# als244/ResNet

Hardware: AMD Instinct MI355X
Metric: images/sec ResNet-50 fp32 224x224 batch256 (higher is better)
Workload: dtype f32

## Files before the change

### include/resnet_mi.h

```cpp
#ifndef RESNET_MI_H
#define RESNET_MI_H
#include <stddef.h>
#include <stdint.h>

#ifdef __cplusplus
extern "C" {
#endif

typedef struct {
    char **labels;
    char **synsets;
    int *counts;
    int n_classes;
} Class_Metadata;

typedef struct {
    int input;
    int init_kernel_dim;
    int init_conv_filters;
    int init_conv_stride;
    int init_maxpool_dim;
    int init_maxpool_stride;
    int n_conv_blocks;
    int *is_block_spatial_reduction;
// ... 218 lines not shown
int mi_op_avgpool_fwd(const float *x, float *y, int N, int C, int H);
int mi_op_avgpool_bwd(const float *dy, float *dx, int N, int C, int H);
int mi_op_relu_deriv(const float *x, const float *up, float *out, size_t n);
int mi_op_matmul(const float *A, const float *B, float *out, int m, int k, int n);
int mi_op_matmul_lt(const float *A_kxm, const float *B, float *out, int m, int k, int n);
int mi_op_matmul_rt(const float *A, const float *B_nxk, float *out, int m, int k, int n);
int mi_op_softmax(const float *x, float *out, int N, int L);
int mi_op_ce_deriv(const float *pred, const int *labels, float *d, int N, int L);
int mi_op_adam(float *p, const float *g, float *m, float *v, size_t n, float lr, float wd, float b1, float b2,
               float cur_b1, float cur_b2, float eps, int *nan_flag_dev);
int mi_op_nhwc_to_nchw(const float *in, float *out, int N, int H, int W, int C);
int mi_debug_lds_fill(uint32_t word);
int mi_debug_poison_lds(void);
int mi_debug_lds_probe(uint32_t word, size_t out[4]);
int mi_debug_lds_geometry(size_t out[3]);
int mi_debug_lds_fill_mode(int on, uint32_t word);
size_t mi_debug_lds_fills(void);
int mi_debug_redzone(size_t zone_bytes, int fill_byte);
int mi_debug_redzone_check(void);
void mi_debug_redzone_stats(size_t *allocs_checked, size_t *zone_bytes_checked, size_t *live);
int mi_debug_trace_names(char *buf, size_t cap);
void mi_debug_trace_clear(void);
int mi_debug_conv_plan(int op, int N, int C, int H, int K, int k, int stride, int out[9]);
int mi_op_fill_uniform(float *out, size_t n, uint64_t seed, float lo, float hi);
enum { MI_ROUTE_DEFAULT = 0, MI_ROUTE_CL = 1, MI_ROUTE_CL2 = 2, MI_ROUTE_PW = 3 };
int mi_conv_plan(int dtype, int route, int op, int N, int C, int H, int K, int k, int stride, int out[7]);
enum { MI_FWD_F32, MI_FWD_BF16, MI_FWD_CL, MI_FWD_STEM_F32, MI_FWD_STEM_BF16, MI_FWD_PW  };
enum { MI_DG_F32, MI_DG_BF16, MI_DG_CL, MI_DG_CL2 };
enum { MI_WG_F32, MI_WG_BF16, MI_WG_CL, MI_WG_CL2, MI_WG_STEM_F32, MI_WG_STEM_BF16 };
int mi_layer_routes(int dtype, int policy, int N, int C, int H, int K, int k, int stride, int site, int out[4]);
enum {
    MI_K_NONE,
    MI_K_IGEMM,
    MI_K_GEMM1X1,
    MI_K_DCONV,
    MI_K_WGRADC,
    MI_K_WGRAD,
    MI_K_BGEMM,
    MI_K_PW_WGRAD,
    MI_K_CL_CONV,
    MI_K_CL_DGRAD2,
    MI_K_CL_WGRAD,
    MI_K_CL_WGRAD2,
    MI_K_ST32_FWD,
    MI_K_ST32_WGRAD,
    MI_K_ST_FWD,
// ... 183 lines not shown
```

### resnet_amd/binding.py

```python
import ctypes as C
import os

_HERE = os.path.dirname(os.path.abspath(__file__))
LIB_PATH = os.environ.get("RESNET_MI_LIB") or os.path.join(_HERE, "libresnet_mi.so")

_fp = C.POINTER(C.c_float)
_ip = C.POINTER(C.c_int)


class Dims(C.Structure):
    _fields_ = [("input", C.c_int), ("init_kernel_dim", C.c_int), ("init_conv_filters", C.c_int),
                ("init_conv_stride", C.c_int), ("init_maxpool_dim", C.c_int), ("init_maxpool_stride", C.c_int),
                ("n_conv_blocks", C.c_int), ("is_block_spatial_reduction", _ip), ("final_depth", C.c_int),
                ("output", C.c_int)]


class BatchNorm(C.Structure):
    _fields_ = [("spatial_dim", C.c_int), ("depth", C.c_int), ("gamma", _fp), ("beta", _fp)]


class ConvBlock(C.Structure):
    _fields_ = [("incoming_filters", C.c_int), ("incoming_spatial_dim", C.c_int), ("reduced_depth", C.c_int),
                ("expanded_depth", C.c_int), ("stride", C.c_int), ("depth_reduction", _fp),
                ("norm_depth_reduction", C.POINTER(BatchNorm)), ("spatial", _fp), ("norm_spatial", C.POINTER(BatchNorm)),
# ... 202 lines not shown
    "mi_op_avgpool_bwd": (_i, [_vp, _vp, _i, _i, _i]),
    "mi_op_relu_deriv": (_i, [_vp, _vp, _vp, _sz]),
    "mi_op_matmul": (_i, [_vp, _vp, _vp, _i, _i, _i]),
    "mi_op_matmul_lt": (_i, [_vp, _vp, _vp, _i, _i, _i]),
    "mi_op_matmul_rt": (_i, [_vp, _vp, _vp, _i, _i, _i]),
    "mi_op_softmax": (_i, [_vp, _vp, _i, _i]),
    "mi_op_ce_deriv": (_i, [_vp, _vp, _vp, _i, _i]),
    "mi_op_adam": (_i, [_vp, _vp, _vp, _vp, _sz, _f, _f, _f, _f, _f, _f, _f, _vp]),
    "mi_op_nhwc_to_nchw": (_i, [_vp, _vp, _i, _i, _i, _i]),
    "mi_op_fill_uniform": (_i, [_vp, _sz, _u64, _f, _f]),
    "mi_debug_poison_lds": (_i, []),
    "mi_debug_lds_fill": (_i, [C.c_uint32]),
    "mi_debug_lds_probe": (_i, [C.c_uint32, C.POINTER(_sz)]),
    "mi_debug_lds_geometry": (_i, [C.POINTER(_sz)]),
    "mi_debug_lds_fill_mode": (_i, [_i, C.c_uint32]),
    "mi_debug_lds_fills": (_sz, []),
    "mi_debug_redzone": (_i, [_sz, _i]),
    "mi_debug_redzone_check": (_i, []),
    "mi_debug_redzone_stats": (None, [C.POINTER(_sz)] * 3),
    "mi_debug_trace_names": (_i, [C.c_char_p, _sz]),
    "mi_debug_trace_clear": (None, []),
    "mi_debug_conv_plan": (_i, [_i] * 7 + [_vp]),
    "mi_conv_plan": (_i, [_i] * 9 + [_vp]),
    "mi_layer_routes": (_i, [_i] * 9 + [_vp]),
    "mi_layer_kernels": (_i, [_i] * 9 + [_vp]),
    "mi_debug_trainer_routes": (_i, [_T, _vp, _i]),
    "mi_trainer_set_dtype": (_i, [_T, _i]),
    "mi_trainer_get_dtype": (_i, [_T]),
    "mi_trainer_set_store_policy": (_i, [_T, _i]),
    "mi_trainer_activation_bytes": (_sz, [_T]),
    "mi_trainer_device_bytes": (_sz, [_T]),
    "mi_clear_error": (None, []),
    "mi_trainer_check_errors": (_i, [_T]),
    "mi_trainer_end_epoch": (None, [_T, _f, _f, _f]),
    "mi_trainer_set_optimizer": (_i, [_T, _i, _f, _f]),
    "mi_trainer_get_optimizer": (_i, [_T]),
    "mi_op_loss_head": (_i, [_vp, _vp, _vp, _vp, _vp, _vp, _i, _i, _f, _i, _vp, _vp]),
    "mi_trainer_set_loss": (_i, [_T, _f, _i, _i]),
    "mi_trainer_metrics": (_i, [_T, C.POINTER(MiLossMetrics), C.POINTER(MiLossMetrics), _i]),
    "mi_trainer_track_running_stats": (_i, [_T, _i, _f]),
    "mi_bn_unbias": (_f, [C.c_int64]),
    "mi_op_bn_running_update": (_i, [_vp, _vp, _vp, _vp, _i, _vp, _i, _f]),
    "mi_trainer_running_stats_channels": (_i, [_T]),
    "mi_trainer_get_running_stats": (_i, [_T, _vp, _vp]),
    "mi_trainer_set_running_stats": (_i, [_T, _vp, _vp]),
    "mi_trainer_running_updates": (C.c_int64, [_T]),
# ... 117 lines not shown
```

### resnet_amd/csrc/kernels_igemm.hip

```cpp
#include "mi_common.hpp"
#include <type_traits>
#include "mi_device.h"

typedef float f32x16 __attribute__((ext_vector_type(16)));
typedef float pf4 __attribute__((ext_vector_type(4)));

enum { IG_FWD = 0, IG_DGRAD = 1, IG_WGRAD = 2 };

struct IgArgs {
    int N, C, K, H, W, Ho, Wo;
    int HW, P;
    int ncols;
    int mtiles;
    int tiles;
    int ctiles;
    int klen;
    FastDiv fdP, fdWo, fdM;
    int full, tsplit, tklen, cpt;
    FastDiv fdTs, fdCpt;
    float *tailbuf;
    float *bn_part;
    int bn_np;
    const float *bnb_x, *bnb_mask, *bnb_mean;
    float *bnb_part;
// ... 21 lines not shown
    if (nv <= 0) { mean = 0.f; m2 = 0.f; }
}
__device__ __forceinline__ void ig_merge(float &na, float &ma, float &qa, float nb, float mb, float qb) {
    const float n = na + nb;
    if (n > 0.f) {
        const float dlt = mb - ma, f = nb / n;
        ma = ma + dlt * f;
        qa = qa + qb + dlt * dlt * na * f;
    }
    na = n;
}

#define IG_BK 32
#ifdef IG_STAMP
__device__ unsigned long long ig_stamps[8 * 16384];
#define IG_T(slot) do { if (threadIdx.x == 0 && blockIdx.x < 16384 && blockIdx.y == 0) ig_stamps[blockIdx.x * 8 + (slot)] = __builtin_amdgcn_s_memtime(); } while (0)
#else
#define IG_T(slot) do { } while (0)
#endif
#ifndef IG_ABLATE
#define IG_ABLATE 0
#endif

template <int MODE, int KS, int S, int WMW, bool VBP = false>
__global__ void __launch_bounds__(256)
igemm_kernel(const float *__restrict__ Aop, const float *__restrict__ Bop, float *__restrict__ Out,
             const float *__restrict__ addend, const IgArgs g) {
    constexpr int BM = 64 * WMW;
    constexpr int TN = WMW == 2 ? 2 : 1;
    constexpr int WNC = 32 * TN;
    constexpr int T = KS * KS, PAD = KS / 2;
    constexpr int LDA = (MODE == IG_WGRAD) ? BM + 1 : BM + 4;
    constexpr int LDB = (MODE == IG_WGRAD) ? 129 : 132;
    constexpr int NA4 = BM / 32;
    constexpr int NAS = BM / 8;
    constexpr bool VB = VBP && KS == 1 && MODE != IG_WGRAD;
    constexpr bool CT64 = VBP && MODE == IG_WGRAD;
    extern __shared__ __attribute__((aligned(16))) float ig_smem[];
    float *As = ig_smem;
    float *Bs = ig_smem + 2 * IG_BK * LDA;
    const int tid = threadIdx.x, lane = tid & 63;
    const int wave = __builtin_amdgcn_readfirstlane(tid >> 6);
    const int wm = WMW == 2 ? wave >> 1 : 0, wn = WMW == 2 ? wave & 1 : wave;

    IG_T(0);
    uint32_t L = blockIdx.x;
    int tail_id = -1, it0 = 0, nt_slice = 0;
    uint32_t wg_split = blockIdx.y;
    if (MODE != IG_WGRAD && g.tsplit > 1 && L >= (uint32_t)g.full) {
        tail_id = (int)(L - (uint32_t)g.full);
        const uint32_t tl = fd_div((uint32_t)tail_id, g.fdTs);
        const int z = tail_id - (int)tl * g.tsplit;
        L = (uint32_t)g.full + tl;
        it0 = z * g.tklen;
        nt_slice = g.tklen;
    } else if (MODE == IG_WGRAD && gridDim.y >= 8) {
        const uint32_t T_ = gridDim.x, tot = T_ * gridDim.y, per = tot >> 3;
        uint32_t V = blockIdx.y * T_ + blockIdx.x;
        if (V < per * 8) V = (V & 7) * per + (V >> 3);
        wg_split = V / T_;
        L = V - wg_split * T_;
    } else {
        const uint32_t lim = MODE != IG_WGRAD && g.tsplit > 1 ? (uint32_t)g.full : (uint32_t)g.tiles;
// ... 7 lines not shown
    f32x16 acc[2][TN];
#pragma unroll
    for (int i = 0; i < 2; i++)
#pragma unroll
        for (int j = 0; j < TN; j++)
#pragma unroll
            for (int r = 0; r < 16; r++) acc[i][j][r] = 0.f;

    uint32_t a_lane = 0, b_lane = 0;
    uint32_t mask = 0;
    int ph = 0, pw = 0, ntaps = 1;
    int wg_t = 0, wg_r = 0, wg_s = 0, cblk = 0, kend = 0;
    int ntiles = 0;
    if (MODE == IG_FWD || MODE == IG_DGRAD) {
        const int Mdim = MODE == IG_FWD ? g.K : g.C;
        const int a_i = (tid & (BM / 4 - 1)) * 4, a_k = tid / (BM / 4);
        a_lane = (uint32_t)(a_k * Mdim + a_i) * 4u;
        const int j = VB ? n0 + (tid & 31) * 4 : n0 + (tid & 127);
        const bool jin = j < g.ncols;
        const uint32_t jc = jin ? (uint32_t)j : (uint32_t)g.ncols - (VB ? 4u : 1u);
        const uint32_t n = fd_div(jc, g.fdP);
        const uint32_t p = jc - n * g.P;
        const uint32_t ho = fd_div(p, g.fdWo), wo = p - ho * g.Wo;
        const int b_k = VB ? (tid >> 5) : 16 * (tid >> 7);
        if (MODE == IG_FWD) {
            b_lane = (uint32_t)(n * g.C * g.HW + (S * ho) * g.W + S * wo + b_k * g.HW) * 4u;
#pragma unroll
            for (int t = 0; t < T; t++) {
                const int hi = S * (int)ho - PAD + t / KS, wi = S * (int)wo - PAD + t % KS;
                if (jin && hi >= 0 && hi < g.H && wi >= 0 && wi < g.W) mask |= 1u << t;
            }
            ntaps = T;
            ntiles = T * (g.C / IG_BK);
        } else if (S == 1) {
            b_lane = (uint32_t)(n * g.K * g.P + p + b_k * g.P) * 4u;
#pragma unroll
            for (int t = 0; t < T; t++) {
                const int hs = (int)ho + PAD - t / KS, ws = (int)wo + PAD - t % KS;
                if (jin && hs >= 0 && hs < g.Ho && ws >= 0 && ws < g.Wo) mask |= 1u << t;
            }
            ntaps = T;
            ntiles = T * (g.K / IG_BK);
        } else {
            const int cls = 3 - (int)blockIdx.y;
            ph = cls >> 1; pw = cls & 1;
            const int ntw = pw ? 2 : 1;
            ntaps = (ph ? 2 : 1) * ntw;
            b_lane = (uint32_t)(n * g.K * g.P + p + b_k * g.P) * 4u;
            for (int tt = 0; tt < ntaps; tt++) {
                const int th = tt / ntw, tw = tt - th * ntw;
                const int dh = (ph && th == 0) ? 1 : 0, dw = (pw && tw == 0) ? 1 : 0;
                if (jin && (int)ho + dh < g.Ho && (int)wo + dw < g.Wo) mask |= 1u << tt;
            }
            ntiles = ntaps * (g.K / IG_BK);
        }
    } else {
        if (CT64) { wg_t = 2 * (int)ct; cblk = 0; }
        else {
            wg_t = (int)(ct / (uint32_t)g.ctiles);
            cblk = (int)(ct - (uint32_t)wg_t * g.ctiles) * 128;
        }
        wg_r = wg_t / KS; wg_s = wg_t - KS * wg_r;
        const int kbeg = (int)wg_split * g.klen;
        kend = min(g.N * g.P, kbeg + g.klen);
        ntiles = (kend - kbeg + IG_BK - 1) / IG_BK;
    }

    pf4 ra4[NA4];
    float ra[NAS], rb[16];
    pf4 rb4[4];
    int sel_a = 1, sel_b = 1;
    int ld_t = 0, ld_c0 = 0;
    if (MODE != IG_WGRAD && tail_id >= 0) {
        ld_t = (int)fd_div((uint32_t)it0, g.fdCpt);
        ld_c0 = (it0 - ld_t * g.cpt) * IG_BK;
        ntiles = min(nt_slice, ntiles - it0);
    }
    int ld_k0 = (MODE == IG_WGRAD) ? (int)wg_split * g.klen : 0;
    const char *fa = nullptr, *fb = nullptr;
    uint32_t fa_lane = 0, fb_lane = 0;
    uint32_t fb_lane2 = 0;
    auto ldg = [](const char *ubase, uint32_t lane_off) -> float { return *(const float *)(ubase + lane_off); };
    auto ldg4 = [](const char *ubase, uint32_t lane_off) -> pf4 { return *(const pf4 *)(ubase + lane_off); };

    auto fetch_into = [&](const int p, pf4 *ra4, float *ra, float *rb, pf4 *rb4, int &sel_a, int &sel_b) {
        if (MODE == IG_FWD || MODE == IG_DGRAD) {
            if (p == 0) {
                const int t = min(ld_t, ntaps - 1);
                sel_b = (mask >> t) & 1;
                if (MODE == IG_FWD) {
                    const int r = KS == 3 ? (t * 11) >> 5 : 0, s = t - KS * r;
                    fa = (const char *)(Aop + (size_t)(t * g.C + ld_c0) * g.K + m0);
                    fb = (const char *)(Bop + (size_t)ld_c0 * g.HW);
                    fb_lane = b_lane + (uint32_t)(sel_b * ((r - PAD) * g.W + (s - PAD)) * 4);
                    ld_c0 += IG_BK;
                    if (ld_c0 == g.C) { ld_c0 = 0; ld_t++; }
                } else {
                    int wt, doff;
                    if (S == 1) {
                        const int r = KS == 3 ? (t * 11) >> 5 : 0, s = t - KS * r;
                        wt = t;
                        doff = (PAD - r) * g.Wo + (PAD - s);
                    } else {
                        const int th = pw ? t >> 1 : t, tw = pw ? t & 1 : 0;
                        const int r = ph ? 2 * th : 1, s = pw ? 2 * tw : 1;
                        wt = 3 * r + s;
                        doff = (ph & (th ^ 1)) * g.Wo + (pw & (tw ^ 1));
                    }
                    fa = (const char *)(Aop + (size_t)(wt * g.K + ld_c0) * g.C + m0);
                    fb = (const char *)(Bop + (size_t)ld_c0 * g.P);
                    fb_lane = b_lane + (uint32_t)(sel_b * doff * 4);
                    ld_c0 += IG_BK;
                    if (ld_c0 == g.K) { ld_c0 = 0; ld_t++; }
                }
            }
            const size_t bstride = (MODE == IG_FWD ? (size_t)g.HW : (size_t)g.P) * 4;
            const size_t astride = (MODE == IG_FWD ? (size_t)g.K : (size_t)g.C) * 4;
            if (VB) { if ((p & 1) == 0) rb4[p >> 1] = ldg4(fb + (size_t)(4 * p) * bstride, fb_lane); }
            else {
                rb[2 * p] = ldg(fb + (size_t)(2 * p) * bstride, fb_lane);
                rb[2 * p + 1] = ldg(fb + (size_t)(2 * p + 1) * bstride, fb_lane);
            }
            if (p % (8 / NA4) == 0) ra4[p / (8 / NA4)] = ldg4(fa + (size_t)(4 * p) * astride, a_lane);
        } else {
            if (p == 0) {
                const int kk = ld_k0 + (tid & 31);
                sel_a = kk < kend;
                const uint32_t kc = sel_a ? (uint32_t)kk : (uint32_t)kend - 1;
                const uint32_t n = fd_div_ge2(kc, g.fdP);
                const uint32_t pp = kc - n * g.P;
                const uint32_t ho = fd_div_ge2(pp, g.fdWo), wo = pp - ho * g.Wo;
                const int hi = S * (int)ho - PAD + wg_r, wi = S * (int)wo - PAD + wg_s;
                const int inb = (int)((uint32_t)hi < (uint32_t)g.H) & (int)((uint32_t)wi < (uint32_t)g.W);
                sel_b = sel_a & inb;
                const uint32_t row = (uint32_t)tid >> 5;
                fa = (const char *)(Aop + (size_t)m0 * g.P);
                fb = (const char *)(Bop + (size_t)cblk * g.HW);
                fa_lane = (n * (uint32_t)(g.K * g.P) + pp + row * g.P) * 4u;
                const uint32_t pix = inb ? (uint32_t)(hi * g.W + wi) : (S * ho) * g.W + S * wo;
                fb_lane = (n * (uint32_t)(g.C * g.HW) + pix + row * g.HW) * 4u;
                if (CT64) {
                    const int t1 = wg_t + 1, r1 = t1 / KS, s1 = t1 - KS * r1;
                    const int hj = S * (int)ho - PAD + r1, wj = S * (int)wo - PAD + s1;
                    const int inb1 = (int)((uint32_t)hj < (uint32_t)g.H) & (int)((uint32_t)wj < (uint32_t)g.W) & (int)(t1 < T);
                    const uint32_t pix1 = inb1 ? (uint32_t)(hj * g.W + wj) : (S * ho) * g.W + S * wo;
                    fb_lane2 = (n * (uint32_t)(g.C * g.HW) + pix1 + row * g.HW) * 4u;
                    sel_b |= (sel_a & inb1) << 1;
                }
                ld_k0 += IG_BK;
            }
            if (NAS == 16) {
                ra[2 * p] = ldg(fa + (size_t)(16 * p) * g.P * 4, fa_lane);
                ra[2 * p + 1] = ldg(fa + (size_t)(16 * p + 8) * g.P * 4, fa_lane);
            } else ra[p] = ldg(fa + (size_t)(8 * p) * g.P * 4, fa_lane);
            if (CT64) {
                rb[2 * p] = ldg(fb + (size_t)(16 * (p & 3)) * g.HW * 4, p < 4 ? fb_lane : fb_lane2);
                rb[2 * p + 1] = ldg(fb + (size_t)(16 * (p & 3) + 8) * g.HW * 4, p < 4 ? fb_lane : fb_lane2);
            } else {
                rb[2 * p] = ldg(fb + (size_t)(16 * p) * g.HW * 4, fb_lane);
                rb[2 * p + 1] = ldg(fb + (size_t)(16 * p + 8) * g.HW * 4, fb_lane);
            }
        }
    };
    auto fetch_part = [&](const int p) { fetch_into(p, ra4, ra, rb, rb4, sel_a, sel_b); };
    auto stash_from = [&](const int buf, const int p, const pf4 *ra4, const float *ra, const float *rb, const pf4 *rb4, const int sel_a, const int sel_b) {
        float *as = As + buf * IG_BK * LDA, *bs = Bs + buf * IG_BK * LDB;
        if (MODE == IG_WGRAD) {
            const int kx = tid & 31, row = tid >> 5;
            if (NAS == 16) {
                as[kx * LDA + row + 16 * p] = sel_a ? ra[2 * p] : 0.f;
                as[kx * LDA + row + 16 * p + 8] = sel_a ? ra[2 * p + 1] : 0.f;
            } else as[kx * LDA + row + 8 * p] = sel_a ? ra[p] : 0.f;
            const int sb = CT64 ? (sel_b >> (p >> 2)) & 1 : sel_b;
            bs[kx * LDB + row + 16 * p] = sb ? rb[2 * p] : 0.f;
            bs[kx * LDB + row + 16 * p + 8] = sb ? rb[2 * p + 1] : 0.f;
        } else {
            if (VB) {
                if ((p & 1) == 0) {
                    const pf4 z = {0.f, 0.f, 0.f, 0.f};
                    *(pf4 *)(bs + ((tid >> 5) + 4 * p) * LDB + (tid & 31) * 4) = sel_b ? rb4[p >> 1] : z;
                }
            } else {
                const int bj = tid & 127, b_k = 16 * (tid >> 7);
                bs[(b_k + 2 * p) * LDB + bj] = sel_b ? rb[2 * p] : 0.f;
                bs[(b_k + 2 * p + 1) * LDB + bj] = sel_b ? rb[2 * p + 1] : 0.f;
            }
            if (p % (8 / NA4) == 0) {
                const int a_i = (tid & (BM / 4 - 1)) * 4, a_k = tid / (BM / 4);
                *(pf4 *)(as + (a_k + 4 * p) * LDA + a_i) = ra4[p / (8 / NA4)];
            }
        }
    };
    auto stash_part = [&](const int buf, const int p) { stash_from(buf, p, ra4, ra, rb, rb4, sel_a, sel_b); };

    const int fr = lane & 31, fk = lane >> 5;
    {
        pf4 pa4[NA4], pb4[4];
        float pa[NAS], pb[16];
        int psel_a = 1, psel_b = 1;
#pragma unroll
        for (int p = 0; p < 8; p++) fetch_into(p, pa4, pa, pb, pb4, psel_a, psel_b);
#pragma unroll
        for (int p = 0; p < 8; p++) fetch_part(p);
#pragma unroll
        for (int p = 0; p < 8; p++) stash_from(0, p, pa4, pa, pb, pb4, psel_a, psel_b);
    }
    if (MODE == IG_WGRAD) {
#pragma unroll
        for (int q = 0; q < NAS; q++) asm volatile("" : "+v"(ra[q]));
    } else {
#pragma unroll
        for (int q = 0; q < NA4; q++) asm volatile("" : "+v"(ra4[q]));
    }
#pragma unroll
    for (int q = 0; q < 16; q++) { if (!VB) asm volatile("" : "+v"(rb[q])); }
#pragma unroll
    for (int q = 0; q < 4; q++) { if (VB) asm volatile("" : "+v"(rb4[q])); }
    __syncthreads();
    IG_T(1);
    auto kstep = [&](auto st_tag, auto ft_tag, const int buf) {
        constexpr bool st = IG_ABLATE != 1 && decltype(st_tag)::value;
        constexpr bool ft = IG_ABLATE != 1 && IG_ABLATE != 4 && decltype(ft_tag)::value;
        const float *as = As + buf * IG_BK * LDA + fk * LDA + wm * 64 + fr;
        const float *bs = Bs + buf * IG_BK * LDB + fk * LDB + wn * WNC + fr;
        float av[2][2], bv[2][TN];
#pragma unroll
        for (int i = 0; i < 2; i++) av[0][i] = as[i * 32];
#pragma unroll
        for (int j = 0; j < TN; j++) bv[0][j] = bs[j * 32];
#pragma unroll
        for (int k2 = 0; k2 < IG_BK; k2 += 2) {
            const int cur = (k2 >> 1) & 1, grp = k2 >> 1;
            if (k2 + 2 < IG_BK) {
#pragma unroll
                for (int i = 0; i < 2; i++) av[cur ^ 1][i] = as[(k2 + 2) * LDA + i * 32];
#pragma unroll
                for (int j = 0; j < TN; j++) bv[cur ^ 1][j] = bs[(k2 + 2) * LDB + j * 32];
            }
            __builtin_amdgcn_sched_barrier(0);
            if (grp < 8) { if (st) stash_part(buf ^ 1, grp); }
            else { if (ft) fetch_part(grp - 8); }
#pragma unroll
            for (int i = 0; i < 2; i++)
#pragma unroll
                for (int j = 0; j < TN; j++)
                    acc[i][j] = __builtin_amdgcn_mfma_f32_32x32x2f32(av[cur][i], bv[cur][j], acc[i][j], 0, 0, 0);
            __builtin_amdgcn_sched_barrier(0);
        }
        __syncthreads();
    };
    {
        constexpr std::true_type Y{};
        constexpr std::false_type NO{};
        int it = 0;
        for (; it + 2 < ntiles; it++) kstep(Y, Y, it & 1);
        if (it + 1 < ntiles) { kstep(Y, NO, it & 1); it++; }
        if (it < ntiles) kstep(NO, NO, it & 1);
    }

    IG_T(2);
    if (MODE != IG_WGRAD && tail_id >= 0) {
        float *tb = g.tailbuf + (size_t)tail_id * (BM * 128);
#pragma unroll
        for (int j = 0; j < TN; j++)
#pragma unroll
            for (int i = 0; i < 2; i++)
#pragma unroll
                for (int r = 0; r < 16; r++)
                    tb[(wm * 64 + i * 32 + (r & 3) + 8 * (r >> 2) + 4 * (lane >> 5)) * 128 + wn * WNC + j * 32 + (lane & 31)] = acc[i][j][r];
        return;
    }
    if (MODE == IG_DGRAD && S == 1 && g.bnb_part) {
        constexpr int PPT = 4 / WMW;
        if ((g.P & 3) == 0) {
            constexpr int CPR = WNC / 4, RPI = 64 / CPR, PITCH = WNC + 4;
            float *img = ig_smem + wave * (32 * PITCH);
            const int c4 = (lane % CPR) * 4, r0 = lane / CPR;
            const int col = n0 + wn * WNC + c4;
            const bool cok = col < g.ncols;
            const uint32_t jc = cok ? (uint32_t)col : 0u;
// ... 480 lines not shown
        const int splits = igemm_wgrad_splits(N, K, H, C, 1, 1);
        igemm_geometry(g, N,  K, H,  C, 1);
        bm = C % 128 == 0 ? 128 : 64;
        g.mtiles = C / bm;
        g.ctiles = K / 128;
        g.tiles = g.mtiles * g.ctiles;
        g.klen = mi_cdiv(mi_cdiv(N * g.P, splits), IG_BK) * IG_BK;
    } else {
        const int T = k * k;
        const int splits = igemm_wgrad_splits(N, C, H, K, k, stride);
        igemm_geometry(g, N, C, H, K, stride);
        bm = K % 128 == 0 ? 128 : 64;
        g.mtiles = K / bm;
        g.ctiles = C / 128;
        g.tiles = C == 64 ? g.mtiles * ((T + 1) / 2) : g.mtiles * T * g.ctiles;
        g.klen = mi_cdiv(mi_cdiv(N * g.P, splits), IG_BK) * IG_BK;
    }
    g.fdM = make_fastdiv(g.mtiles);
    g.full = g.tiles; g.tsplit = 1; g.fdTs = make_fastdiv(1); g.cpt = 1; g.fdCpt = make_fastdiv(1);
    *used = mi_cdiv(N * g.P, g.klen);
    return bm;
}
static thread_local const char *ig_variant = "igemm_kernel";
template <int MODE, int KS, int S, int WMW, bool VB = false>
static int igemm_launch_t(hipStream_t st, dim3 grid, const float *A, const float *B, float *out, const float *addend, const IgArgs &g) {
    constexpr int BM = 64 * WMW;
    constexpr int LDA = (MODE == IG_WGRAD) ? BM + 1 : BM + 4, LDB = (MODE == IG_WGRAD) ? 129 : 132;
    constexpr size_t lds = (size_t)2 * IG_BK * (LDA + LDB) * sizeof(float);
    static int attr_set = 0;
    if (!attr_set) {
        if (lds > 64 * 1024 &&
            hipFuncSetAttribute((const void *)igemm_kernel<MODE, KS, S, WMW, VB>, hipFuncAttributeMaxDynamicSharedMemorySize, (int)lds) != hipSuccess) {
            mi_record_error("igemm_kernel", "cannot raise the dynamic LDS limit");
            return -1;
        }
        attr_set = 1;
    }
    hipLaunchKernelGGL((igemm_kernel<MODE, KS, S, WMW, VB>), grid, dim3(256), lds, st, A, B, out, addend, g);
    ig_variant = mi_trace_name("igemm_kernel<%s,k%d,s%d,bm%d%s%s>", MODE == IG_FWD ? "fwd" : MODE == IG_DGRAD ? "dgrad" : "wgrad", KS, S, BM, VB ? ",vb" : "",
                               g.tsplit > 1 ? ",tail" : "");
    return 0;
}
template <int MODE>
static int igemm_launch(hipStream_t st, dim3 grid, const float *A, const float *B, float *out, const float *addend, const IgArgs &g,
                        int k, int stride, int bm) {
#define IGL(KS_, S_)                                                                                      \
    if (k == KS_ && stride == S_)                                                                         \
        return bm == 128 ? igemm_launch_t<MODE, KS_, S_, 2>(st, grid, A, B, out, addend, g)               \
                         : igemm_launch_t<MODE, KS_, S_, 1>(st, grid, A, B, out, addend, g);
    if (MODE != IG_WGRAD && k == 1 && stride == 1 && g.P % 4 == 0)
        return bm == 128 ? igemm_launch_t<MODE, 1, 1, 2, true>(st, grid, A, B, out, addend, g)
                         : igemm_launch_t<MODE, 1, 1, 1, true>(st, grid, A, B, out, addend, g);
    if (MODE == IG_WGRAD && k == 3 && g.C == 64) {
        if (stride == 1) return bm == 128 ? igemm_launch_t<MODE, 3, 1, 2, true>(st, grid, A, B, out, addend, g) : igemm_launch_t<MODE, 3, 1, 1, true>(st, grid, A, B, out, addend, g);
        return bm == 128 ? igemm_launch_t<MODE, 3, 2, 2, true>(st, grid, A, B, out, addend, g) : igemm_launch_t<MODE, 3, 2, 1, true>(st, grid, A, B, out, addend, g);
    }
    IGL(1, 1) IGL(3, 1) IGL(3, 2)
#undef IGL
    return -2;
}
static int igemm_fam(int k) { return k == 1 ? MI_FAM_GEMM : MI_FAM_PCONV; }

extern "C" int mi_igemm_fwd(mid_stream s, mid_workspace *ws, const float *x, const float *w, float *y, int N, int C, int H, int K, int k,
                            int stride, mid_bn_parts *parts) {
    hipStream_t st = (hipStream_t)s;
    const int T = k * k;
    if (parts) parts->nparts = 0;
    if (!mi_igemm_supported(IGOP_FWD, N, C, H, K, k, stride)) { mi_record_error("mi_igemm_fwd", "shape not supported by the implicit GEMM"); return -2; }
    if (!ws || ws->wt_floats < (size_t)T * C * K) { mi_record_error("mi_igemm_fwd", "workspace too small"); return -3; }
    const float *A = ws->pre_fwd;
    if (!A) {
        if (k == 1) hipLaunchKernelGGL(igemm_wt_kernel<1>, dim3(C / 32, K / 32), dim3(256), 0, st, w, ws->wt, K, C, 1);
        else hipLaunchKernelGGL(igemm_wt_kernel<9>, dim3(C / 32, K / 32), dim3(256), 0, st, w, ws->wt, K, C, 1);
        MI_LAUNCH_CHECK("igemm_wt_kernel");
        A = ws->wt;
    }
    IgArgs g = {};
    const int bm = igemm_plan_tiles(g, IGOP_FWD, N, C, H, K, k, stride);
    igemm_tail_plan(g, T * g.cpt, ws->wt_floats >= (size_t)T * C * K + IG_TAIL_FLOATS ? ws->wt + (size_t)T * C * K : nullptr, bm);
    if (parts) {
        parts->nparts = 0;
        const int np = mi_cdiv(g.ncols, 128) * (bm == 128 ? 2 : 4);
// ... 101 lines not shown
extern "C" int mi_debug_igemm_stamps(unsigned long long *dst, int nblocks) {
    return hipMemcpyFromSymbol(dst, HIP_SYMBOL(ig_stamps), sizeof(unsigned long long) * 8 * (size_t)nblocks) == hipSuccess ? 0 : -1;
}
#endif

extern "C" int mid_igemm_plan(int op, int N, int C, int H, int K, int k, int stride, int out[9]) {
    for (int i = 0; i < 9; i++) out[i] = 0;
    if (!mi_igemm_supported(op, N, C, H, K, k, stride)) return 0;
    out[0] = 1;
    IgArgs g = {};
    if (op == IGOP_WGRAD) {
        int used;
        out[1] = igemm_plan_wgrad(g, N, C, H, K, k, stride, igemm_wgrad_swapped(C, K, k), &used);
        out[2] = g.tiles; out[3] = g.tiles; out[4] = 1; out[5] = g.klen / IG_BK; out[6] = used; out[7] = g.tiles; out[8] = mi_cdiv(N * g.P, IG_BK);
        return 1;
    }
    const int bm = igemm_plan_tiles(g, op, N, C, H, K, k, stride);
    float dummy;
    igemm_tail_plan(g, k * k * g.cpt, (op == IGOP_FWD || stride == 1) ? &dummy : nullptr, bm);
    out[1] = bm; out[2] = g.tiles; out[3] = g.full; out[4] = g.tsplit; out[5] = g.tklen; out[6] = 1;
    out[7] = g.full + (g.tiles - g.full) * g.tsplit; out[8] = k * k * g.cpt;
    return 1;
}
extern "C" int mid_wgrad_reduce_grouped(int K, int C, int splits) { return igemm_wgrad_reduce_grouped((long)K * C, splits) ? 1 : 0; }
extern "C" int mid_igemm_conv_plan(int op, int N, int C, int H, int K, int k, int stride, int out[7]) {
    int o[9];
    if (!mid_igemm_plan(op, N, C, H, K, k, stride, o)) return 0;
    out[0] = o[1]; out[1] = 128; out[2] = o[2]; out[3] = o[3]; out[4] = o[4]; out[5] = o[6];
    out[6] = op == IGOP_WGRAD && !igemm_wgrad_swapped(C, K, k) ? mid_wgrad_reduce_grouped(K, C, o[6]) : 0;
    return 1;
}

extern "C" int mid_conv_prelayout_all(mid_stream s, const mid_wt_entry *entries_dev, const int *tile_entry_dev, int ntiles) {
    if (ntiles <= 0) return 0;
    hipLaunchKernelGGL(igemm_wt_all_kernel, dim3(ntiles), dim3(256), 0, (hipStream_t)s, entries_dev, tile_entry_dev);
    MI_LAUNCH_CHECK("igemm_wt_all_kernel");
    return 0;
}
```

### resnet_amd/csrc/mi_device.h

```cpp
#ifndef MI_DEVICE_H
#define MI_DEVICE_H
#include <stddef.h>
#include <stdint.h>
#ifdef __cplusplus
extern "C" {
#endif

typedef void *mid_stream;
typedef void *mid_event;

enum { MID_F32 = 0, MID_BF16 = 1 };

int mid_device_count(void);
int mid_set_device(int dev);
const char *mid_last_error(void);
void mid_clear_error(void);
void *mid_malloc(size_t bytes);
void mid_free(void *p);
int mid_redzone(size_t zone_bytes, int fill_byte);
int mid_redzone_check(void);
void mid_redzone_stats(size_t *allocs_checked, size_t *zone_bytes_checked, size_t *live);
int mid_trace_names(char *buf, size_t cap);
void mid_trace_clear(void);
void *mid_malloc_host(size_t bytes);
// ... 106 lines not shown
int mid_cl_wgrad(mid_stream s, const void *xp, const void *dy, float *dw, float *part, size_t part_floats, int N, int C, int H, int K, int stride);
int mid_cl_dgrad2_supported(int N, int C, int H, int K);
size_t mid_cl_dgrad2_operand_bytes(int N, int K, int Ho);
int mid_cl_relayout_end(mid_stream s, const void *dy, void *dyp, int N, int K, int Ho);
int mid_cl_dgrad2(mid_stream s, const void *dyp, const void *a_tiles, void *dx, int N, int C, int H, int K);
size_t mid_stem_f32_xp_bytes(int N, int H);
int mid_stem_fwd_f32(mid_stream s, const float *x, const float *w, float *y, void *xp, size_t xp_bytes, float *scratch, size_t scratch_floats,
                     int N, int H, mid_bn_parts *parts);
int mid_stem_wgrad_f32(mid_stream s, const void *xp, const float *dy, float *dw, float *scratch, size_t scratch_floats, int N, int H);
int mid_stem_bf16_supported(int C, int H, int K, int k, int stride);
size_t mid_stem_bf16_xp_bytes(int N, int H);
size_t mid_stem_bf16_part_floats(int N, int H);
int mid_stem_fwd_bf16(mid_stream s, const float *x, const float *w, void *y, int y_dt, void *xp, size_t xp_bytes, float *scratch, size_t scratch_floats,
                      int N, int H, mid_bn_parts *parts);
int mid_stem_wgrad_bf16(mid_stream s, const void *xp, const void *dy, int dy_dt, float *dw, float *scratch, size_t scratch_floats, int N, int H);
int mid_f32_to_bf16(mid_stream s, const float *in, void *out, size_t n);
int mid_bf16_to_f32(mid_stream s, const void *in, float *out, size_t n);

int mid_igemm_plan(int op, int N, int C, int H, int K, int k, int stride, int out[9]);
int mid_igemm_conv_plan(int op, int N, int C, int H, int K, int k, int stride, int out[7]);
int mid_bf16_conv_plan(int op, int N, int C, int H, int K, int k, int stride, int out[7]);
int mid_cl_conv_plan(int route, int op, int N, int C, int H, int K, int k, int stride, int out[7]);
int mid_wgrad_reduce_grouped(int K, int C, int splits);

int mid_gemm_nn(mid_stream s, const float *A, const float *B, float *out, int m, int k, int n);
int mid_gemm_tn(mid_stream s, const float *At, const float *B, float *out, int m, int k, int n);
int mid_gemm_nt(mid_stream s, const float *A, const float *Bt, float *out, int m, int k, int n);

size_t mid_bn_ws_floats(int C);
int mid_bn_fwd(mid_stream s, float *stats_ws, const float *x, const float *gamma, const float *beta,
               const float *residual, float *means, float *vars, float *y, float *xhat_out, float *norm_out, int N,
               int C, int P, float eps, int relu);
int mid_bn_fwd_parts(mid_stream s, float *stats_ws, const mid_bn_parts *parts, const float *x, const float *gamma,
                     const float *beta, const float *residual, float *means, float *vars, float *y, float *xhat_out,
                     float *norm_out, int N, int C, int P, float eps, int relu);
int mid_bn_bwd(mid_stream s, float *stats_ws, const float *x, const float *gamma, const float *beta,
               const float *means, const float *vars, const float *dy, const float *mask_src, float *dx,
               float *dgamma, float *dbeta, int N, int C, int P, float eps, int mask_mode);

int mid_bn_bwd_gate(mid_stream s, float *stats_ws, const float *x, const float *gamma, const float *beta,
                    const float *means, const float *vars, const float *dy, const float *mask_src, float *gated_out,
                    float *dx, float *dgamma, float *dbeta, int N, int C, int P, float eps);

int mid_bn_fwd_t(mid_stream s, float *stats_ws, const mid_bn_parts *parts, const void *x, int x_dt, const float *gamma,
                 const float *beta, const void *residual, float *means, float *vars, void *y, int a_dt, float *xhat_out,
                 float *norm_out, int N, int C, int P, float eps, int relu, void *ycl, int Hcl);
// ... 91 lines not shown
```

### resnet_amd/csrc/ops.c

```c
#include <math.h>
#include <stdint.h>
#include <stdlib.h>
#include <string.h>
#include "mi_host.h"

void *mi_malloc(size_t bytes) {
    char *p = (char *)mid_malloc(bytes + 2 * MI_GUARD);
    return p ? p + MI_GUARD : NULL;
}
void mi_free(void *p) { if (p) mid_free((char *)p - MI_GUARD); }

static int finish(int rc) {
    mid_stream_sync(mi_global()->compute);
    if (rc) return rc;
    return mid_last_error()[0] ? -1 : 0;
}

typedef struct { MiLayer L; MiLayerWs w; mid_wt_entry we; mid_stream s; int rc; } OpConv;
static MiOptions op_options(void) {
    MiOptions env, o = {.bnfuse_bwd = 1, .bnfuse_bwd_f32 = 7};
    mi_read_options(&env);
    o.igemm = env.igemm; o.pw_wgrad = env.pw_wgrad;
    return o;
}
// ... 284 lines not shown
}
void mi_debug_ta_geometry(size_t out[4]) { mid_ta_geometry(out); }
int mi_op_fill_uniform(float *out, size_t n, uint64_t seed, float lo, float hi) { return finish(mid_fill_uniform(mi_global()->compute, out, n, seed, 0, lo, hi)); }
int mi_debug_lds_fill(uint32_t word) { return finish(mid_debug_lds_fill(word)); }
int mi_debug_poison_lds(void) { return mi_debug_lds_fill(0xFFFFFFFFu); }
int mi_debug_lds_probe(uint32_t word, size_t out[4]) { return finish(mid_debug_lds_probe(word, out)); }
int mi_debug_lds_geometry(size_t out[3]) { return finish(mid_debug_lds_geometry(out)); }
int mi_debug_lds_fill_mode(int on, uint32_t word) { return finish(mid_debug_lds_fill_mode(on, word)); }
size_t mi_debug_lds_fills(void) { return mid_debug_lds_fills(); }
int mi_debug_redzone(size_t zone_bytes, int fill_byte) { return mid_redzone(zone_bytes, fill_byte); }
int mi_debug_redzone_check(void) { return mid_redzone_check(); }
void mi_debug_redzone_stats(size_t *allocs_checked, size_t *zone_bytes_checked, size_t *live) { mid_redzone_stats(allocs_checked, zone_bytes_checked, live); }
int mi_debug_trace_names(char *buf, size_t cap) { return mid_trace_names(buf, cap); }
void mi_debug_trace_clear(void) { mid_trace_clear(); }
static int on_igemm(int op, int N, int C, int H, int K, int k, int stride) {
    const MiOptions opt = op_options();
    return op >= 0 && op <= 2 && mi_layer_f32_kernel(&opt, op, N, C, H, K, k, stride) == MI_K_IGEMM;
}
int mi_debug_conv_plan(int op, int N, int C, int H, int K, int k, int stride, int out[9]) {
    if (on_igemm(op, N, C, H, K, k, stride)) return mid_igemm_plan(op, N, C, H, K, k, stride, out);
    for (int i = 0; i < 9; i++) out[i] = 0;
    return 0;
}
int mi_conv_plan(int dtype, int route, int op, int N, int C, int H, int K, int k, int stride, int out[7]) {
    for (int i = 0; i < 7; i++) out[i] = 0;
    int ok = 0;
    if (op < 0 || op > 2) ok = 0;
    else if (dtype == MI_DTYPE_F32 && route == MI_ROUTE_DEFAULT) ok = on_igemm(op, N, C, H, K, k, stride) && mid_igemm_conv_plan(op, N, C, H, K, k, stride, out);
    else if (dtype == MI_DTYPE_BF16 && route == MI_ROUTE_DEFAULT) ok = mid_bf16_conv_plan(op, N, C, H, K, k, stride, out);
    else if (dtype == MI_DTYPE_BF16 && route >= MI_ROUTE_CL && route <= MI_ROUTE_PW) ok = mid_cl_conv_plan(route, op, N, C, H, K, k, stride, out);
    if (!ok) { for (int i = 0; i < 7; i++) out[i] = 0; return -2; }
    return 0;
}

int mi_op_convert(const void *in, int in_dt, void *out, int out_dt, size_t n) {
    if (in_dt == MID_F32 && out_dt == MID_BF16) return finish(mid_f32_to_bf16(mi_global()->compute, (const float *)in, out, n));
    if (in_dt == MID_BF16 && out_dt == MID_F32) return finish(mid_bf16_to_f32(mi_global()->compute, in, (float *)out, n));
    return -2;
}
int mi_op_conv_fwd_bf16(const void *x, const float *w, void *y, int N, int C, int H, int K, int k, int stride) {
    return op_conv(MID_BF16, MI_FWD_BF16, OFF, OFF, x, w, NULL, y, NULL, N, C, H, K, k, stride);
}
int mi_op_conv_dgrad_bf16(const float *w, const void *dy, void *dx, int N, int C, int H, int K, int k, int stride, int to_add) {
    return op_conv(MID_BF16, OFF, MI_DG_BF16, OFF, NULL, w, dy, dx, to_add ? dx : NULL, N, C, H, K, k, stride);
}
int mi_op_conv_wgrad_bf16(const void *x, const void *dy, float *dw, int N, int C, int H, int K, int k, int stride) {
// ... 154 lines not shown
```

Measured before the change: 2428.

## Use half-depth K staging for 3x3 dgrad 128-wide igemm tiles to raise occupancy

Templates the implicit-GEMM conv kernel on its staged K depth (16 or 32) and generalizes all fetch/stash index math accordingly. The planner selects depth 16 for 3x3 dgrad with 128-wide tiles, with higher launch-bound minimum waves for reduced-depth variants and LDS sized to cover the epilogue buffers. The intent is to cut LDS and register footprint so more waves fit per CU, at the cost of twice as many K steps and barriers. A debug override and a query function are exposed.

After: 2443 (median of 6 runs). No clear change (+0.6%).

```diff
diff --git a/include/resnet_mi.h b/include/resnet_mi.h
--- a/include/resnet_mi.h
+++ b/include/resnet_mi.h
@@ -264,6 +264,8 @@
 int mi_debug_trace_names(char *buf, size_t cap);
 void mi_debug_trace_clear(void);
 int mi_debug_conv_plan(int op, int N, int C, int H, int K, int k, int stride, int out[9]);
+int mi_debug_igemm_depth(int depth);
+int mi_debug_igemm_plan_depth(int op, int N, int C, int H, int K, int k, int stride);
 int mi_op_fill_uniform(float *out, size_t n, uint64_t seed, float lo, float hi);
 enum { MI_ROUTE_DEFAULT = 0, MI_ROUTE_CL = 1, MI_ROUTE_CL2 = 2, MI_ROUTE_PW = 3 };
 int mi_conv_plan(int dtype, int route, int op, int N, int C, int H, int K, int k, int stride, int out[7]);
diff --git a/resnet_amd/binding.py b/resnet_amd/binding.py
--- a/resnet_amd/binding.py
+++ b/resnet_amd/binding.py
@@ -248,6 +248,8 @@
     "mi_debug_trace_clear": (None, []),
     "mi_debug_conv_plan": (_i, [_i] * 7 + [_vp]),
     "mi_conv_plan": (_i, [_i] * 9 + [_vp]),
+    "mi_debug_igemm_depth": (_i, [_i]),
+    "mi_debug_igemm_plan_depth": (_i, [_i] * 7),
     "mi_layer_routes": (_i, [_i] * 9 + [_vp]),
     "mi_layer_kernels": (_i, [_i] * 9 + [_vp]),
     "mi_debug_trainer_routes": (_i, [_T, _vp, _i]),
diff --git a/resnet_amd/csrc/kernels_igemm.hip b/resnet_amd/csrc/kernels_igemm.hip
--- a/resnet_amd/csrc/kernels_igemm.hip
+++ b/resnet_amd/csrc/kernels_igemm.hip
@@ -67,8 +67,9 @@
 #define IG_ABLATE 0
 #endif
 
-template <int MODE, int KS, int S, int WMW, bool VBP = false>
-__global__ void __launch_bounds__(256)
+constexpr int ig_min_waves(int mode, int s, int wmw, int bk) { return bk == IG_BK ? 1 : (mode == IG_DGRAD && s == 1 && wmw == 2) ? 2 : 3; }
+template <int MODE, int KS, int S, int WMW, bool VBP = false, int BK = IG_BK>
+__global__ void __launch_bounds__(256, ig_min_waves(MODE, S, WMW, BK))
 igemm_kernel(const float *__restrict__ Aop, const float *__restrict__ Bop, float *__restrict__ Out,
              const float *__restrict__ addend, const IgArgs g) {
     constexpr int BM = 64 * WMW;
@@ -77,13 +78,17 @@
     constexpr int T = KS * KS, PAD = KS / 2;
     constexpr int LDA = (MODE == IG_WGRAD) ? BM + 1 : BM + 4;
     constexpr int LDB = (MODE == IG_WGRAD) ? 129 : 132;
-    constexpr int NA4 = BM / 32;
-    constexpr int NAS = BM / 8;
+    constexpr int NP = BK / 4, LBK = BK == 32 ? 5 : 4;
+    constexpr int RG = 256 / BK;
+    constexpr int NA4 = BM * BK / 1024;
+    constexpr int NAS = BM * BK / 256;
+    constexpr int NB = BK / 2, NB4 = BK / 8;
+    static_assert(BK == 32 || BK == 16, "staged depth");
     constexpr bool VB = VBP && KS == 1 && MODE != IG_WGRAD;
     constexpr bool CT64 = VBP && MODE == IG_WGRAD;
     extern __shared__ __attribute__((aligned(16))) float ig_smem[];
     float *As = ig_smem;
-    float *Bs = ig_smem + 2 * IG_BK * LDA;
+    float *Bs = ig_smem + 2 * BK * LDA;
     const int tid = threadIdx.x, lane = tid & 63;
     const int wave = __builtin_amdgcn_readfirstlane(tid >> 6);
     const int wm = WMW == 2 ? wave >> 1 : 0, wn = WMW == 2 ? wave & 1 : wave;
@@ -137,7 +142,7 @@
         const uint32_t n = fd_div(jc, g.fdP);
         const uint32_t p = jc - n * g.P;
         const uint32_t ho = fd_div(p, g.fdWo), wo = p - ho * g.Wo;
-        const int b_k = VB ? (tid >> 5) : 16 * (tid >> 7);
+        const int b_k = VB ? (tid >> 5) : NB * (tid >> 7);
         if (MODE == IG_FWD) {
             b_lane = (uint32_t)(n * g.C * g.HW + (S * ho) * g.W + S * wo + b_k * g.HW) * 4u;
 #pragma unroll
@@ -182,8 +187,8 @@
     }
 
     pf4 ra4[NA4];
-    float ra[NAS], rb[16];
-    pf4 rb4[4];
+    float ra[NAS], rb[NB];
+    pf4 rb4[NB4];
     int sel_a = 1, sel_b = 1;
     int ld_t = 0, ld_c0 = 0;
     if (MODE != IG_WGRAD && tail_id >= 0) {
@@ -208,7 +213,7 @@
                     fa = (const char *)(Aop + (size_t)(t * g.C + ld_c0) * g.K + m0);
                     fb = (const char *)(Bop + (size_t)ld_c0 * g.HW);
                     fb_lane = b_lane + (uint32_t)(sel_b * ((r - PAD) * g.W + (s - PAD)) * 4);
-                    ld_c0 += IG_BK;
+                    ld_c0 += BK;
                     if (ld_c0 == g.C) { ld_c0 = 0; ld_t++; }
                 } else {
                     int wt, doff;
@@ -225,7 +230,7 @@
                     fa = (const char *)(Aop + (size_t)(wt * g.K + ld_c0) * g.C + m0);
                     fb = (const char *)(Bop + (size_t)ld_c0 * g.P);
                     fb_lane = b_lane + (uint32_t)(sel_b * doff * 4);
-                    ld_c0 += IG_BK;
+                    ld_c0 += BK;
                     if (ld_c0 == g.K) { ld_c0 = 0; ld_t++; }
                 }
             }
@@ -236,10 +241,10 @@
                 rb[2 * p] = ldg(fb + (size_t)(2 * p) * bstride, fb_lane);
                 rb[2 * p + 1] = ldg(fb + (size_t)(2 * p + 1) * bstride, fb_lane);
             }
-            if (p % (8 / NA4) == 0) ra4[p / (8 / NA4)] = ldg4(fa + (size_t)(4 * p) * astride, a_lane);
+            if (p % (NP / NA4) == 0) ra4[p / (NP / NA4)] = ldg4(fa + (size_t)(4 * p) * astride, a_lane);
         } else {
             if (p == 0) {
-                const int kk = ld_k0 + (tid & 31);
+                const int kk = ld_k0 + (tid & (BK - 1));
                 sel_a = kk < kend;
                 const uint32_t kc = sel_a ? (uint32_t)kk : (uint32_t)kend - 1;
                 const uint32_t n = fd_div_ge2(kc, g.fdP);
@@ -248,7 +253,7 @@
                 const int hi = S * (int)ho - PAD + wg_r, wi = S * (int)wo - PAD + wg_s;
                 const int inb = (int)((uint32_t)hi < (uint32_t)g.H) & (int)((uint32_t)wi < (uint32_t)g.W);
                 sel_b = sel_a & inb;
-                const uint32_t row = (uint32_t)tid >> 5;
+                const uint32_t row = (uint32_t)tid >> LBK;
                 fa = (const char *)(Aop + (size_t)m0 * g.P);
                 fb = (const char *)(Bop + (size_t)cblk * g.HW);
                 fa_lane = (n * (uint32_t)(g.K * g.P) + pp + row * g.P) * 4u;
@@ -262,33 +267,34 @@
                     fb_lane2 = (n * (uint32_t)(g.C * g.HW) + pix1 + row * g.HW) * 4u;
                     sel_b |= (sel_a & inb1) << 1;
                 }
-                ld_k0 += IG_BK;
-            }
-            if (NAS == 16) {
-                ra[2 * p] = ldg(fa + (size_t)(16 * p) * g.P * 4, fa_lane);
-                ra[2 * p + 1] = ldg(fa + (size_t)(16 * p + 8) * g.P * 4, fa_lane);
-            } else ra[p] = ldg(fa + (size_t)(8 * p) * g.P * 4, fa_lane);
+                ld_k0 += BK;
+            }
+            if (BM == 128) {
+                ra[2 * p] = ldg(fa + (size_t)(2 * RG * p) * g.P * 4, fa_lane);
+                ra[2 * p + 1] = ldg(fa + (size_t)(2 * RG * p + RG) * g.P * 4, fa_lane);
+            } else ra[p] = ldg(fa + (size_t)(RG * p) * g.P * 4, fa_lane);
             if (CT64) {
-                rb[2 * p] = ldg(fb + (size_t)(16 * (p & 3)) * g.HW * 4, p < 4 ? fb_lane : fb_lane2);
-                rb[2 * p + 1] = ldg(fb + (size_t)(16 * (p & 3) + 8) * g.HW * 4, p < 4 ? fb_lane : fb_lane2);
+                constexpr int H = NP / 2;
+                rb[2 * p] = ldg(fb + (size_t)(2 * RG * (p & (H - 1))) * g.HW * 4, p < H ? fb_lane : fb_lane2);
+                rb[2 * p + 1] = ldg(fb + (size_t)(2 * RG * (p & (H - 1)) + RG) * g.HW * 4, p < H ? fb_lane : fb_lane2);
             } else {
-                rb[2 * p] = ldg(fb + (size_t)(16 * p) * g.HW * 4, fb_lane);
-                rb[2 * p + 1] = ldg(fb + (size_t)(16 * p + 8) * g.HW * 4, fb_lane);
+                rb[2 * p] = ldg(fb + (size_t)(2 * RG * p) * g.HW * 4, fb_lane);
+                rb[2 * p + 1] = ldg(fb + (size_t)(2 * RG * p + RG) * g.HW * 4, fb_lane);
             }
         }
     };
     auto fetch_part = [&](const int p) { fetch_into(p, ra4, ra, rb, rb4, sel_a, sel_b); };
     auto stash_from = [&](const int buf, const int p, const pf4 *ra4, const float *ra, const float *rb, const pf4 *rb4, const int sel_a, const int sel_b) {
-        float *as = As + buf * IG_BK * LDA, *bs = Bs + buf * IG_BK * LDB;
+        float *as = As + buf * BK * LDA, *bs = Bs + buf * BK * LDB;
         if (MODE == IG_WGRAD) {
-            const int kx = tid & 31, row = tid >> 5;
-            if (NAS == 16) {
-                as[kx * LDA + row + 16 * p] = sel_a ? ra[2 * p] : 0.f;
-                as[kx * LDA + row + 16 * p + 8] = sel_a ? ra[2 * p + 1] : 0.f;
-            } else as[kx * LDA + row + 8 * p] = sel_a ? ra[p] : 0.f;
-            const int sb = CT64 ? (sel_b >> (p >> 2)) & 1 : sel_b;
-            bs[kx * LDB + row + 16 * p] = sb ? rb[2 * p] : 0.f;
-            bs[kx * LDB + row + 16 * p + 8] = sb ? rb[2 * p + 1] : 0.f;
+            const int kx = tid & (BK - 1), row = tid >> LBK;
+            if (BM == 128) {
+                as[kx * LDA + row + 2 * RG * p] = sel_a ? ra[2 * p] : 0.f;
+                as[kx * LDA + row + 2 * RG * p + RG] = sel_a ? ra[2 * p + 1] : 0.f;
+            } else as[kx * LDA + row + RG * p] = sel_a ? ra[p] : 0.f;
+            const int sb = CT64 ? (sel_b >> (p / (NP / 2))) & 1 : sel_b;
+            bs[kx * LDB + row + 2 * RG * p] = sb ? rb[2 * p] : 0.f;
+            bs[kx * LDB + row + 2 * RG * p + RG] = sb ? rb[2 * p + 1] : 0.f;
         } else {
             if (VB) {
                 if ((p & 1) == 0) {
@@ -296,13 +302,13 @@
                     *(pf4 *)(bs + ((tid >> 5) + 4 * p) * LDB + (tid & 31) * 4) = sel_b ? rb4[p >> 1] : z;
                 }
             } else {
-                const int bj = tid & 127, b_k = 16 * (tid >> 7);
+                const int bj = tid & 127, b_k = NB * (tid >> 7);
                 bs[(b_k + 2 * p) * LDB + bj] = sel_b ? rb[2 * p] : 0.f;
                 bs[(b_k + 2 * p + 1) * LDB + bj] = sel_b ? rb[2 * p + 1] : 0.f;
             }
-            if (p % (8 / NA4) == 0) {
+            if (p % (NP / NA4) == 0) {
                 const int a_i = (tid & (BM / 4 - 1)) * 4, a_k = tid / (BM / 4);
-                *(pf4 *)(as + (a_k + 4 * p) * LDA + a_i) = ra4[p / (8 / NA4)];
+                *(pf4 *)(as + (a_k + 4 * p) * LDA + a_i) = ra4[p / (NP / NA4)];
             }
         }
     };
@@ -310,15 +316,15 @@
 
     const int fr = lane & 31, fk = lane >> 5;
     {
-        pf4 pa4[NA4], pb4[4];
-        float pa[NAS], pb[16];
+        pf4 pa4[NA4], pb4[NB4];
+        float pa[NAS], pb[NB];
         int psel_a = 1, psel_b = 1;
 #pragma unroll
-        for (int p = 0; p < 8; p++) fetch_into(p, pa4, pa, pb, pb4, psel_a, psel_b);
-#pragma unroll
-        for (int p = 0; p < 8; p++) fetch_part(p);
-#pragma unroll
-        for (int p = 0; p < 8; p++) stash_from(0, p, pa4, pa, pb, pb4, psel_a, psel_b);
+        for (int p = 0; p < NP; p++) fetch_into(p, pa4, pa, pb, pb4, psel_a, psel_b);
+#pragma unroll
+        for (int p = 0; p < NP; p++) fetch_part(p);
+#pragma unroll
+        for (int p = 0; p < NP; p++) stash_from(0, p, pa4, pa, pb, pb4, psel_a, psel_b);
     }
     if (MODE == IG_WGRAD) {
 #pragma unroll
@@ -328,33 +334,33 @@
         for (int q = 0; q < NA4; q++) asm volatile("" : "+v"(ra4[q]));
     }
 #pragma unroll
-    for (int q = 0; q < 16; q++) { if (!VB) asm volatile("" : "+v"(rb[q])); }
-#pragma unroll
-    for (int q = 0; q < 4; q++) { if (VB) asm volatile("" : "+v"(rb4[q])); }
+    for (int q = 0; q < NB; q++) { if (!VB) asm volatile("" : "+v"(rb[q])); }
+#pragma unroll
+    for (int q = 0; q < NB4; q++) { if (VB) asm volatile("" : "+v"(rb4[q])); }
     __syncthreads();
     IG_T(1);
     auto kstep = [&](auto st_tag, auto ft_tag, const int buf) {
         constexpr bool st = IG_ABLATE != 1 && decltype(st_tag)::value;
         constexpr bool ft = IG_ABLATE != 1 && IG_ABLATE != 4 && decltype(ft_tag)::value;
-        const float *as = As + buf * IG_BK * LDA + fk * LDA + wm * 64 + fr;
-        const float *bs = Bs + buf * IG_BK * LDB + fk * LDB + wn * WNC + fr;
+        const float *as = As + buf * BK * LDA + fk * LDA + wm * 64 + fr;
+        const float *bs = Bs + buf * BK * LDB + fk * LDB + wn * WNC + fr;
         float av[2][2], bv[2][TN];
 #pragma unroll
         for (int i = 0; i < 2; i++) av[0][i] = as[i * 32];
 #pragma unroll
         for (int j = 0; j < TN; j++) bv[0][j] = bs[j * 32];
 #pragma unroll
-        for (int k2 = 0; k2 < IG_BK; k2 += 2) {
+        for (int k2 = 0; k2 < BK; k2 += 2) {
             const int cur = (k2 >> 1) & 1, grp = k2 >> 1;
-            if (k2 + 2 < IG_BK) {
+            if (k2 + 2 < BK) {
 #pragma unroll
                 for (int i = 0; i < 2; i++) av[cur ^ 1][i] = as[(k2 + 2) * LDA + i * 32];
 #pragma unroll
                 for (int j = 0; j < TN; j++) bv[cur ^ 1][j] = bs[(k2 + 2) * LDB + j * 32];
             }
             __builtin_amdgcn_sched_barrier(0);
-            if (grp < 8) { if (st) stash_part(buf ^ 1, grp); }
-            else { if (ft) fetch_part(grp - 8); }
+            if (grp < NP) { if (st) stash_part(buf ^ 1, grp); }
+            else { if (ft) fetch_part(grp - NP); }
 #pragma unroll
             for (int i = 0; i < 2; i++)
 #pragma unroll
@@ -367,10 +373,11 @@
     {
         constexpr std::true_type Y{};
         constexpr std::false_type NO{};
+        const int nst = ntiles * (IG_BK / BK);
         int it = 0;
-        for (; it + 2 < ntiles; it++) kstep(Y, Y, it & 1);
-        if (it + 1 < ntiles) { kstep(Y, NO, it & 1); it++; }
-        if (it < ntiles) kstep(NO, NO, it & 1);
+        for (; it + 2 < nst; it++) kstep(Y, Y, it & 1);
+        if (it + 1 < nst) { kstep(Y, NO, it & 1); it++; }
+        if (it < nst) kstep(NO, NO, it & 1);
     }
 
     IG_T(2);
@@ -897,42 +904,70 @@
     return bm;
 }
 static thread_local const char *ig_variant = "igemm_kernel";
-template <int MODE, int KS, int S, int WMW, bool VB = false>
+template <int MODE, int KS, int S, int WMW, bool VB = false, int BK = IG_BK>
 static int igemm_launch_t(hipStream_t st, dim3 grid, const float *A, const float *B, float *out, const float *addend, const IgArgs &g) {
     constexpr int BM = 64 * WMW;
     constexpr int LDA = (MODE == IG_WGRAD) ? BM + 1 : BM + 4, LDB = (MODE == IG_WGRAD) ? 129 : 132;
-    constexpr size_t lds = (size_t)2 * IG_BK * (LDA + LDB) * sizeof(float);
+    constexpr size_t lds_stage = (size_t)2 * BK * (LDA + LDB) * sizeof(float);
+    constexpr size_t lds_bn = MODE == IG_FWD ? (size_t)4 * (32 * WMW) * 64 * sizeof(float) : 0;
+    constexpr size_t lds_bnb = MODE == IG_DGRAD && S == 1 ? (size_t)4 * 32 * (32 * WMW + 4) * sizeof(float) : 0;
+    static_assert(BK != IG_BK || (lds_stage >= lds_bn && lds_stage >= lds_bnb), "the full-depth tiles hold every epilogue image");
+    size_t lds = lds_stage;
+    if (BK != IG_BK) {
+        if (g.bn_part && lds < lds_bn) lds = lds_bn;
+        if (g.bnb_part && (g.P & 3) == 0 && lds < lds_bnb) lds = lds_bnb;
+    }
     static int attr_set = 0;
     if (!attr_set) {
-        if (lds > 64 * 1024 &&
-            hipFuncSetAttribute((const void *)igemm_kernel<MODE, KS, S, WMW, VB>, hipFuncAttributeMaxDynamicSharedMemorySize, (int)lds) != hipSuccess) {
+        if (lds_stage > 64 * 1024 &&
+            hipFuncSetAttribute((const void *)igemm_kernel<MODE, KS, S, WMW, VB, BK>, hipFuncAttributeMaxDynamicSharedMemorySize, (int)lds_stage) != hipSuccess) {
             mi_record_error("igemm_kernel", "cannot raise the dynamic LDS limit");
             return -1;
         }
         attr_set = 1;
     }
-    hipLaunchKernelGGL((igemm_kernel<MODE, KS, S, WMW, VB>), grid, dim3(256), lds, st, A, B, out, addend, g);
+    hipLaunchKernelGGL((igemm_kernel<MODE, KS, S, WMW, VB, BK>), grid, dim3(256), lds, st, A, B, out, addend, g);
     ig_variant = mi_trace_name("igemm_kernel<%s,k%d,s%d,bm%d%s%s>", MODE == IG_FWD ? "fwd" : MODE == IG_DGRAD ? "dgrad" : "wgrad", KS, S, BM, VB ? ",vb" : "",
                                g.tsplit > 1 ? ",tail" : "");
     return 0;
 }
+template <int MODE, int BK>
+static int igemm_launch_d(hipStream_t st, dim3 grid, const float *A, const float *B, float *out, const float *addend, const IgArgs &g,
+                          int k, int stride, int bm) {
+#define IGL(KS_, S_)                                                                                      \
+    if (k == KS_ && stride == S_)                                                                         \
+        return bm == 128 ? igemm_launch_t<MODE, KS_, S_, 2, false, BK>(st, grid, A, B, out, addend, g)    \
+                         : igemm_launch_t<MODE, KS_, S_, 1, false, BK>(st, grid, A, B, out, addend, g);
+    if constexpr (MODE != IG_WGRAD) {
+        if (k == 1 && stride == 1 && g.P % 4 == 0)
+            return bm == 128 ? igemm_launch_t<MODE, 1, 1, 2, true, BK>(st, grid, A, B, out, addend, g)
+                             : igemm_launch_t<MODE, 1, 1, 1, true, BK>(st, grid, A, B, out, addend, g);
+    } else {
+        if (k == 3 && g.C == 64) {
+            if (stride == 1) return bm == 128 ? igemm_launch_t<MODE, 3, 1, 2, true, BK>(st, grid, A, B, out, addend, g) : igemm_launch_t<MODE, 3, 1, 1, true, BK>(st, grid, A, B, out, addend, g);
+            return bm == 128 ? igemm_launch_t<MODE, 3, 2, 2, true, BK>(st, grid, A, B, out, addend, g) : igemm_launch_t<MODE, 3, 2, 1, true, BK>(st, grid, A, B, out, addend, g);
+        }
+    }
+    IGL(1, 1) IGL(3, 1) IGL(3, 2)
+#undef IGL
+    return -2;
+}
+static int ig_depth_override = 0;
+extern "C" int mid_igemm_set_depth(int depth) {
+    if (depth != 0 && depth != 16 && depth != IG_BK) { mi_record_error("mi_debug_igemm_depth", "depth is 0 (planner), 16 or 32"); return -2; }
+    ig_depth_override = depth;
+    return 0;
+}
+static int igemm_pick_depth(int mode, int k, int bm) {
+    if (ig_depth_override) return ig_depth_override;
+    if (mode == IG_DGRAD && k == 3 && bm == 128) return 16;
+    return IG_BK;
+}
 template <int MODE>
 static int igemm_launch(hipStream_t st, dim3 grid, const float *A, const float *B, float *out, const float *addend, const IgArgs &g,
                         int k, int stride, int bm) {
-#define IGL(KS_, S_)                                                                                      \
-    if (k == KS_ && stride == S_)                                                                         \
-        return bm == 128 ? igemm_launch_t<MODE, KS_, S_, 2>(st, grid, A, B, out, addend, g)               \
-                         : igemm_launch_t<MODE, KS_, S_, 1>(st, grid, A, B, out, addend, g);
-    if (MODE != IG_WGRAD && k == 1 && stride == 1 && g.P % 4 == 0)
-        return bm == 128 ? igemm_launch_t<MODE, 1, 1, 2, true>(st, grid, A, B, out, addend, g)
-                         : igemm_launch_t<MODE, 1, 1, 1, true>(st, grid, A, B, out, addend, g);
-    if (MODE == IG_WGRAD && k == 3 && g.C == 64) {
-        if (stride == 1) return bm == 128 ? igemm_launch_t<MODE, 3, 1, 2, true>(st, grid, A, B, out, addend, g) : igemm_launch_t<MODE, 3, 1, 1, true>(st, grid, A, B, out, addend, g);
-        return bm == 128 ? igemm_launch_t<MODE, 3, 2, 2, true>(st, grid, A, B, out, addend, g) : igemm_launch_t<MODE, 3, 2, 1, true>(st, grid, A, B, out, addend, g);
-    }
-    IGL(1, 1) IGL(3, 1) IGL(3, 2)
-#undef IGL
-    return -2;
+    if (igemm_pick_depth(MODE, k, bm) == 16) return igemm_launch_d<MODE, 16>(st, grid, A, B, out, addend, g, k, stride, bm);
+    return igemm_launch_d<MODE, IG_BK>(st, grid, A, B, out, addend, g, k, stride, bm);
 }
 static int igemm_fam(int k) { return k == 1 ? MI_FAM_GEMM : MI_FAM_PCONV; }
 
@@ -1080,6 +1115,11 @@
     out[7] = g.full + (g.tiles - g.full) * g.tsplit; out[8] = k * k * g.cpt;
     return 1;
 }
+extern "C" int mid_igemm_depth(int op, int N, int C, int H, int K, int k, int stride) {
+    int o[9];
+    if (!mid_igemm_plan(op, N, C, H, K, k, stride, o)) return 0;
+    return igemm_pick_depth(op, k, o[1]);
+}
 extern "C" int mid_wgrad_reduce_grouped(int K, int C, int splits) { return igemm_wgrad_reduce_grouped((long)K * C, splits) ? 1 : 0; }
 extern "C" int mid_igemm_conv_plan(int op, int N, int C, int H, int K, int k, int stride, int out[7]) {
     int o[9];
diff --git a/resnet_amd/csrc/mi_device.h b/resnet_amd/csrc/mi_device.h
--- a/resnet_amd/csrc/mi_device.h
+++ b/resnet_amd/csrc/mi_device.h
@@ -152,6 +152,8 @@
 int mid_bf16_conv_plan(int op, int N, int C, int H, int K, int k, int stride, int out[7]);
 int mid_cl_conv_plan(int route, int op, int N, int C, int H, int K, int k, int stride, int out[7]);
 int mid_wgrad_reduce_grouped(int K, int C, int splits);
+int mid_igemm_set_depth(int depth);
+int mid_igemm_depth(int op, int N, int C, int H, int K, int k, int stride);
 
 int mid_gemm_nn(mid_stream s, const float *A, const float *B, float *out, int m, int k, int n);
 int mid_gemm_tn(mid_stream s, const float *At, const float *B, float *out, int m, int k, int n);
diff --git a/resnet_amd/csrc/ops.c b/resnet_amd/csrc/ops.c
--- a/resnet_amd/csrc/ops.c
+++ b/resnet_amd/csrc/ops.c
@@ -330,6 +330,10 @@
     for (int i = 0; i < 9; i++) out[i] = 0;
     return 0;
 }
+int mi_debug_igemm_depth(int depth) { return mid_igemm_set_depth(depth); }
+int mi_debug_igemm_plan_depth(int op, int N, int C, int H, int K, int k, int stride) {
+    return on_igemm(op, N, C, H, K, k, stride) ? mid_igemm_depth(op, N, C, H, K, k, stride) : 0;
+}
 int mi_conv_plan(int dtype, int route, int op, int N, int C, int H, int K, int k, int stride, int out[7]) {
     for (int i = 0; i < 7; i++) out[i] = 0;
     int ok = 0;
```
